# zwu88/TANTE

Hardware: AMD Instinct MI355X
Metric: rollout frames/sec (fwd), TANTE on 256x256 Active Matter (higher is better)
Workload: dtype bf16

## Files before the change

### include/tante_hip.h

```cpp
#ifndef TANTE_HIP_H
#define TANTE_HIP_H

#include <stddef.h>
#include <stdint.h>

#ifdef __cplusplus
extern "C" {
#endif

#define TANTE_F32 0
#define TANTE_BF16 1

#define TANTE_ACT_NONE 0
#define TANTE_ACT_GELU_ERF 1
#define TANTE_ACT_GELU_TANH 2
#define TANTE_ACT_RELU 3

#define TANTE_A_LINEAR 0
#define TANTE_A_PATCH_NHWC 1
#define TANTE_A_PATCH_NCHW 2

#define TANTE_E_LINEAR 0
#define TANTE_E_FILM 1
#define TANTE_E_DECONV_NHWC 2
// ... 101 lines not shown

int tante_taylor(const float* last, int64_t last_bstride, const float* const* derivs, int n_order, double dt,
                 int n_out, float* out, int64_t out_bstride, int64_t B, int64_t frame, void* stream);

int tante_rt_reduce(const float* t, int B, int L, float out_T, float ep, float* rt, void* stream);

int tante_block_fused_supported(int C, int n_head, int hidden, int L);
int64_t tante_block_stream_bytes(int C, int hidden);
int tante_pack_block(const float* ln1_w, const float* ln1_b, const float* in_w, const float* in_b, const float* out_w,
                     const float* out_b, const float* ln2_w, const float* ln2_b, const float* fc1_w, const float* fc1_b,
                     const float* fc2_w, const float* fc2_b, int C, int hidden, void* block_stream, void* stream);
int tante_block_fused(float* x, const void* block_stream, int C, int n_head, int hidden, const TanteSeq* seq, int causal,
                      float eps, void* stream);
int tante_block_fused_tprop(float* x, const void* block_stream, int C, int n_head, int hidden, const TanteSeq* seq, int causal, float eps,
                            const float* tprop, void* stream);

int tante_set_seed_mix(const uint64_t* device_word);

typedef struct TanteBlockTrain {
  float* out;
  void *xh1, *qkv, *o, *xh2, *hpre, *act;
  float *st1, *x1, *st2;
  float p_drop;
  uint64_t seed_attn, seed_out, seed_mlp;
} TanteBlockTrain;
int tante_pack_block_train(const float* in_w_folded, const float* in_b_folded, const float* out_w, const float* out_b,
                           const float* fc1_w_folded, const float* fc1_b_folded, const float* fc2_w, const float* fc2_b, int C, int hidden,
                           void* block_stream, void* stream);
int tante_block_fused_train(const float* x, const void* block_stream, int C, int n_head, int hidden, const TanteSeq* seq, int causal,
                            float eps, const TanteBlockTrain* tr, void* stream);
// ... 295 lines not shown
```

### tante_amd/_lib.py

```python
import ctypes as C
import os

HERE = os.path.dirname(os.path.abspath(__file__))
LIB_PATH = os.environ.get("TANTE_LIB") or os.path.join(HERE, "lib", "libtante_hip.so")

F32, BF16 = 0, 1
ACT_NONE, ACT_GELU_ERF, ACT_GELU_TANH, ACT_RELU = 0, 1, 2, 3
A_LINEAR, A_PATCH_NHWC, A_PATCH_NCHW = 0, 1, 2
E_LINEAR, E_FILM, E_DECONV_NHWC, E_DECONV_NCHW = 0, 1, 2, 3
W_LINEAR, W_CONV_NHWC, W_DECONV_NHWC, W_DECONV_NCHW = 0, 1, 2, 3
W_LINEAR_T, W_CONV_NHWC_T, W_DECONV_NHWC_T, W_DECONV_NCHW_T = 4, 5, 6, 7

c_i32, c_i64, c_f32, c_vp = C.c_int32, C.c_int64, C.c_float, C.c_void_p


class PackGeom(C.Structure):
    _fields_ = [("n_pad", c_i32), ("k_pad", c_i32), ("nt", c_i32), ("cb", c_i32), ("bytes", c_i64)]


class Gemm(C.Structure):
    _fields_ = [
        ("a", c_vp), ("a_dtype", c_i32), ("a_mode", c_i32), ("M", c_i32), ("K", c_i32),
        ("a_s1", c_i64), ("a_s0", c_i64), ("a_off", c_i64), ("a_n0", c_i32),
        ("Hin", c_i32), ("Win", c_i32), ("Cin", c_i32), ("P", c_i32), ("ln", c_i32), ("ln_eps", c_f32),
# ... 90 lines not shown
    "tante_axis_hw": ([c_vp, c_i64, c_i32, c_i32, c_i32] + [c_vp] * 8 + [c_i32, c_vp], c_i32),
    "tante_axis_hw_film": ([c_vp, c_vp, c_i64, c_i64, c_vp, c_vp, c_vp, c_i32, c_i64, c_i32, c_i32, c_i32] + [c_vp] * 8 + [c_i32, c_vp], c_i32),
    "tante_axis_hw_oop": ([c_vp, c_vp, c_i64, c_i32, c_i32, c_i32, c_vp, c_vp, c_vp, c_vp, c_vp, c_vp, c_vp, c_vp, c_i32, c_vp], c_i32),
    "tante_axis_hw_train": ([c_vp, c_vp, c_vp, c_i64, c_i32, c_i32, c_i32, c_vp, c_vp, c_vp, c_vp, c_vp, c_vp, c_vp, c_vp, c_i32, c_vp], c_i32),
    "tante_film_table": ([c_vp, c_i32, c_i32] + [c_vp] * 8 + [c_vp, c_vp, c_vp, c_vp], c_i32),
    "tante_film_apply": ([c_vp, c_i64, c_vp, c_i64, c_i32, c_i64, c_vp, c_vp, c_vp], c_i32),
    "tante_format_input": ([c_vp, c_i64, c_i32, c_i64, c_i32, c_vp, c_i64, c_vp], c_i32),
    "tante_taylor": ([c_vp, c_i64, C.POINTER(c_vp), c_i32, C.c_double, c_i32, c_vp, c_i64, c_i64, c_i64, c_vp], c_i32),
    "tante_rt_reduce": ([c_vp, c_i32, c_i32, c_f32, c_f32, c_vp, c_vp], c_i32),
    "tante_gather_last": ([c_vp, c_i64, c_i32, c_vp, c_vp], c_i32),
    "tante_block_fused_supported": ([c_i32, c_i32, c_i32, c_i32], c_i32),
    "tante_block_stream_bytes": ([c_i32, c_i32], c_i64),
    "tante_pack_block": ([c_vp] * 12 + [c_i32, c_i32, c_vp, c_vp], c_i32),
    "tante_block_fused": ([c_vp, c_vp, c_i32, c_i32, c_i32, C.POINTER(Seq), c_i32, c_f32, c_vp], c_i32),
    "tante_block_fused_tprop": ([c_vp, c_vp, c_i32, c_i32, c_i32, C.POINTER(Seq), c_i32, c_f32, c_vp, c_vp], c_i32),
    "tante_block_tail_bwd_stream_bytes": ([c_i32, c_i32], c_i64),
    "tante_pack_block_tail_bwd": ([c_vp, c_vp, c_vp, c_i32, c_i32, c_vp, c_vp], c_i32),
    "tante_block_tail_bwd": ([c_vp, c_vp, c_vp, c_vp, c_vp, c_i64, c_i32, c_i32, c_f32, C.c_uint64, C.c_uint64, c_vp, c_vp, c_vp, c_vp, c_vp, c_vp], c_i32),
    "tante_block_head_bwd": ([c_vp, c_vp, c_vp, c_vp, c_vp, c_i64, c_i32, c_vp, c_vp], c_i32),
    "tante_block_bwd_fused_supported": ([c_i32, c_i32, c_i32, c_i32, c_i32], c_i32),
    "tante_block_bwd_fused": ([c_vp] * 9 + [c_i32, c_i32, c_i32, C.POINTER(Seq), c_i32, c_f32, C.c_uint64, C.c_uint64, C.c_uint64] + [c_vp] * 6, c_i32),
    "tante_pack_block_train": ([c_vp] * 8 + [c_i32, c_i32, c_vp, c_vp], c_i32),
    "tante_block_fused_train": ([c_vp, c_vp, c_i32, c_i32, c_i32, C.POINTER(Seq), c_i32, c_f32, C.POINTER(BlockTrain), c_vp], c_i32),
    "tante_head_fused_supported": ([c_i32, c_i32], c_i32),
    "tante_head_stream_bytes": ([c_i32], c_i64),
    "tante_pack_head": ([c_vp] * 6 + [c_i32, c_i32, c_vp, c_vp], c_i32),
    "tante_head_fused": ([c_vp, c_i32, c_i64, c_i64, c_i64, c_i32, c_i32, c_i32, c_i32, c_i32, c_vp, c_vp, c_i64, c_i32, c_vp, c_vp, c_i64, c_vp], c_i32),
    "tante_enc23_supported": ([c_i32], c_i32),
    "tante_enc23_stream_bytes": ([c_i32], c_i64),
    "tante_pack_enc23": ([c_vp] * 4 + [c_i32, c_vp, c_vp], c_i32),
# ... 93 lines not shown
    "tante_pack_head_enc": ([c_vp] * 6 + [c_i32, c_i32, c_vp, c_vp], c_i32),
    "tante_head_enc_fused": ([c_i32, c_vp, c_vp, c_vp, c_i32, c_i64, c_i64, c_i64, c_i32, c_i32, c_i32, c_i32, c_i32, c_vp, c_i64, c_vp, c_i64,
                             c_vp, c_vp, c_vp, c_i64, c_vp], c_i32),
}

LIB_OPTIONS = ("TANTE_ATTN_BWD_HG", "TANTE_ATTN_BWD_NO_SPLIT", "TANTE_ATTN_BWD_VALU", "TANTE_ATTN_FWD_VALU", "TANTE_AXIS_BWD_SMALL_WGS",
               "TANTE_AXIS_BWD_WGS", "TANTE_AXIS_CT", "TANTE_AXIS_FILM", "TANTE_AXIS_GENERIC", "TANTE_AXIS_MFMA", "TANTE_AXIS_NT", "TANTE_AXIS_WGRAD_WGS",
               "TANTE_BLOCK_KERNEL", "TANTE_COLSUM_ROWS", "TANTE_CVIT_CHAIN_TOKENS", "TANTE_ENC23_SPLIT", "TANTE_FILM_BWD_ROWS",
               "TANTE_FS_GROUPS", "TANTE_FS_HALF", "TANTE_FS_SKEW", "TANTE_FS_WAVES", "TANTE_GEMM_NO_LITE", "TANTE_GEMM_SMALLM", "TANTE_GEMM_WGS", "TANTE_HEAD_WAVES",
               "TANTE_IM2COL_TILED", "TANTE_RESIZE_TILED", "TANTE_SPECTRAL_BF16OUT", "TANTE_SPECTRAL_DFT", "TANTE_SPECTRAL_X3", "TANTE_WGRAD_DEEP",
               "TANTE_WGRAD_JOBS", "TANTE_WGRAD_JOBS_WGS", "TANTE_WGRAD_NO_SLAB", "TANTE_WGRAD_NO_TR", "TANTE_WGRAD_REDUCE_NY",
               "TANTE_WGRAD_RG", "TANTE_WGRAD_SLAB_WGS", "TANTE_WGRAD_TR_WGS", "TANTE_WGRAD_WGS", "TANTE_XATTN_GPW", "TANTE_XATTN_VALU",)


_lib = None
ABI_VERSION = 12


def lib():
    global _lib
    if _lib is None:
        if not os.path.exists(LIB_PATH):
            raise RuntimeError(
                f"{LIB_PATH} is missing: build it with `python -m tante_amd.build` "
                "(or __graft_entry__.build()).  tante_amd has no CPU / eager fallback.")
        L = C.CDLL(LIB_PATH)
        for name, (argtypes, restype) in SIGNATURES.items():
            fn = getattr(L, name)
            fn.argtypes = argtypes
            fn.restype = restype
        got = int(L.tante_abi_version())
# ... 32 lines not shown
```

### tante_amd/attn_backbone.py

```python
from __future__ import annotations

import math
import os
from typing import Optional

import torch
import torch.nn as nn

from . import _lib as L
from . import kernels as K
from . import options as _O

FUSE_TPROP = _O.register("TANTE_FUSE_TPROP", True, __name__, "FUSE_TPROP")


def resolve_compute(module_default: Optional[str] = None) -> int:
    if module_default is not None:
        return K.COMPUTE[module_default]
    if torch.is_autocast_enabled("cuda"):
        dt = torch.get_autocast_dtype("cuda")
        if dt == torch.bfloat16:
            return L.BF16
        if dt == torch.float16:
            global _FP16_NOTED
# ... 81 lines not shown
        params = self.__dict__.get("_fused_params")
        if params is None:
            a, m = self.attn, self.mlp
            params = [self.ln1.weight, self.ln1.bias, a.in_proj_weight, a.in_proj_bias, a.out_proj.weight, a.out_proj.bias,
                      self.ln2.weight, self.ln2.bias, m[0].weight, m[0].bias, m[2].weight, m[2].bias]
            self.__dict__["_fused_params"] = params
        return self._cache.get(-1, params, lambda: K.pack_block(params, self.embed_dim, self.hidden))

    def _apply(self, fn, *a, **kw):
        self.__dict__.pop("_fused_params", None)
        return super()._apply(fn, *a, **kw)

    def takes_tprop(self, seq_L: int, compute: int) -> bool:
        return (FUSE_TPROP and compute == L.BF16 and self.fused and self.ln1.eps == self.ln2.eps and seq_L == 4 and self.embed_dim == 256
                and self.n_head == 8 and self.hidden == 256 and not (self.training and self.p_drop > 0.0))

    def forward_tokens(self, x: torch.Tensor, seq: L.Seq, causal: bool, compute: int, tprop: Optional[torch.Tensor] = None) -> torch.Tensor:
        if self.training and self.p_drop > 0.0:
            if tprop is not None:
                raise RuntimeError("TransformerBlock.forward_tokens: tprop is an inference-path fusion (takes_tprop is False under dropout)")
            from .train_forward import block_train
            with torch.no_grad():
                y = block_train(self, x.view(-1, self.embed_dim), seq, causal, compute)
            x.view(-1, self.embed_dim).copy_(y)
            return x
        C_ = self.embed_dim
        n_tok = x.numel() // C_
        if (compute == L.BF16 and self.fused and self.ln1.eps == self.ln2.eps
                and K.block_fused_supported(C_, self.n_head, self.hidden, seq.L)):
            return K.block_fused(x, self._packed_fused(), C_, self.n_head, self.hidden, seq, causal, self.ln1.eps, tprop)
# ... 116 lines not shown
        tp = self.temporal_propagator
        params = [tp[0].weight, tp[0].bias, tp[2].weight, tp[2].bias]
        return self._tp_cache.get(0, params, lambda: torch.cat([p.detach().float().reshape(-1) for p in params]).contiguous())

    def _packed_channel(self, compute: int):
        params = [p for cb in self.channel_blocks for p in cb.parameters()]

        def build():
            return [(K.pack_weight(cb[0].weight, cb[0].bias, compute), K.pack_weight(cb[2].weight, cb[2].bias, compute))
                    for cb in self.channel_blocks]
        return self._cache.get(compute, params, build)

    def takes_x_in(self, compute: int) -> bool:
        return K.axis_hw_train_supported(self.H, self.W, self.C, compute)

    def forward_tokens(self, x: torch.Tensor, B: int, compute: int, film_src: Optional[tuple] = None, x_in: Optional[torch.Tensor] = None,
                       film_frames: Optional[tuple] = None) -> torch.Tensor:
        T, H, W, C_ = self.T, self.H, self.W, self.C
        vp, hp, tp = self.vertical_propagator, self.horizontal_propagator, self.temporal_propagator
        if film_frames is not None:
            import ctypes as C
            fr, _keep, fa, fb, se = film_frames
            L.check(L.lib().tante_axis_mlp_film(x.data_ptr(), C.byref(fr), fa.data_ptr(), fb.data_ptr(), se.data_ptr(), B, T, H, W * C_, C_,
                                                vp[0].weight.data_ptr(), vp[0].bias.data_ptr(), vp[2].weight.data_ptr(), vp[2].bias.data_ptr(),
                                                K._stream()), "tante_axis_mlp_film")
            K.axis_mlp(x, B * T * H, W, C_, hp[0].weight, hp[0].bias, hp[2].weight, hp[2].bias, compute)
        elif x_in is not None:
            K.axis_hw_oop(x_in, x, B * T, H, W, C_, (vp[0].weight, vp[0].bias, vp[2].weight, vp[2].bias),
                          (hp[0].weight, hp[0].bias, hp[2].weight, hp[2].bias), compute)
        elif film_src is not None:
            z, ts, bs, film = film_src
            K.axis_hw_film(x, z, ts, bs, film, B * T, H, W, C_, (vp[0].weight, vp[0].bias, vp[2].weight, vp[2].bias),
                           (hp[0].weight, hp[0].bias, hp[2].weight, hp[2].bias), compute)
        elif K.axis_hw_supported(H, W, C_, compute):
            K.axis_hw(x, B * T, H, W, C_, (vp[0].weight, vp[0].bias, vp[2].weight, vp[2].bias),
                      (hp[0].weight, hp[0].bias, hp[2].weight, hp[2].bias), compute)
        else:
            K.axis_mlp(x, B * T, H, W * C_, vp[0].weight, vp[0].bias, vp[2].weight, vp[2].bias, compute)
            K.axis_mlp(x, B * T * H, W, C_, hp[0].weight, hp[0].bias, hp[2].weight, hp[2].bias, compute)
        tprop = None
        if (T == 4 and len(self.attn_axes) > 0 and self.attn_axes[0] == "T" and not torch.is_grad_enabled()
                and self.blocks[0].takes_tprop(T, compute)):
            tprop = self._packed_tprop()
        else:
            K.axis_mlp(x, B, T, H * W * C_, tp[0].weight, tp[0].bias, tp[2].weight, tp[2].bias, compute)
        ci = 0
        for i, axis in enumerate(self.attn_axes):
            blk = self.blocks[i]
            if axis == "C":
                E = self.expanded_channel
                lift1, lift2 = self._packed_channel(compute)[ci]
                ci += 1
                n = x.numel()
                adt = K.act_torch_dtype(compute)
                z1 = torch.empty(n, E // 4, dtype=adt, device=x.device)
                K.linear(x, lift1, z1, M=n, act=L.ACT_GELU_ERF, a_s0=1)
                z = torch.empty(n, E, dtype=torch.float32, device=x.device)
                K.linear(z1, lift2, z, M=n)
                blk.forward_tokens(z, K.dense_seq(n // C_, C_), False, compute)
                K.gather_last(z, n, E, x)
            else:
                blk.forward_tokens(x, K.make_seq(axis, B, T, H, W), axis == "T", compute, tprop if i == 0 else None)
        return x

# ... 12 lines not shown
```

### tante_amd/csrc/block_fused.hip

```cpp
#include "common.hip.h"

#include <stdlib.h>
#include "fused_common.hip.h"
#include "block_sliced.h"

namespace {

constexpr int BIAS_BYTES = 4096;

__device__ __forceinline__ long seq_token(const TanteSeq& q, int s, int l) {
  return (long)(s / q.n_s0) * q.S1 + (long)(s % q.n_s0) * q.S0 + (long)(l / q.n_l0) * q.P1 + (long)(l % q.n_l0) * q.P0;
}

template <int BYTES>
__device__ __forceinline__ void glds_copy(const char* __restrict__ g, char* l, int tid) {
  static_assert(BYTES % 4096 == 0, "tiles are whole LDS-DMA passes");
  const int wave = tid >> 6, lane = tid & 63;
#pragma unroll
  for (int i = 0; i < BYTES / 4096; ++i) {
    const int off = i * 4096 + wave * 1024;
    __builtin_amdgcn_global_load_lds((const __attribute__((address_space(1))) void*)(g + off + lane * 16),
                                     (__attribute__((address_space(3))) void*)(l + off), 16, 0, 0);
  }
}
// ... 676 lines not shown
  return 0;
}

extern "C" int tante_block_fused_tprop(float* x, const void* block_stream, int C, int n_head, int hidden, const TanteSeq* seq, int causal, float eps,
                                       const float* tprop, void* stream) {
  if (!x || !block_stream || !seq || !tprop) TANTE_FAIL(-1, "tante_block_fused_tprop: null pointer");
  if (seq->L != 4 || !tante_block_fused_supported(C, n_head, hidden, seq->L) || !use_fs(C, n_head, hidden, seq->L, causal))
    TANTE_FAIL(-2, "tante_block_fused_tprop: the feature-sliced kernel at L = 4 only (C=%d heads=%d hidden=%d L=%d)", C, n_head, hidden, seq->L);
  if (((uintptr_t)x % 16) || ((uintptr_t)block_stream % 16)) TANTE_FAIL(-1, "tante_block_fused_tprop: buffers must be 16-byte aligned");
  if (tante_fs_launch(x, (const char*)block_stream + block_ts_stream_bytes(C, hidden), *seq, causal, eps, (hipStream_t)stream, nullptr, tprop) != 0)
    TANTE_FAIL(-2, "tante_block_fused_tprop: too many sequences (%d)", seq->nseq);
  TANTE_CHECK_LAUNCH();
  return 0;
}

extern "C" int tante_block_fused(float* x, const void* block_stream, int C, int n_head, int hidden, const TanteSeq* seq, int causal,
                                 float eps, void* stream) {
  if (!x || !block_stream || !seq) TANTE_FAIL(-1, "tante_block_fused: null pointer");
  if (!tante_block_fused_supported(C, n_head, hidden, seq->L))
    TANTE_FAIL(-2, "tante_block_fused: unsupported shape C=%d heads=%d hidden=%d L=%d", C, n_head, hidden, seq->L);
  if (((uintptr_t)x % 16) || ((uintptr_t)block_stream % 16)) TANTE_FAIL(-1, "tante_block_fused: buffers must be 16-byte aligned");
  hipStream_t s = (hipStream_t)stream;
  const char* st = (const char*)block_stream;
  if (use_fs(C, n_head, hidden, seq->L, causal)) {
    if (tante_fs_launch(x, st + block_ts_stream_bytes(C, hidden), *seq, causal, eps, s) != 0)
      TANTE_FAIL(-2, "tante_block_fused: too many sequences (%d)", seq->nseq);
    TANTE_CHECK_LAUNCH();
    return 0;
  }
  const int key = (C / 32) * 100 + hidden / 32;
// ... 60 lines not shown
```

### tante_amd/csrc/block_sliced.h

```cpp
#pragma once
#include <hip/hip_runtime.h>
#include <stdint.h>
#include "../../include/tante_hip.h"

int tante_fs_supported(int C, int n_head, int hidden, int L, int causal);
int64_t tante_fs_stream_bytes(int C, int hidden);
void tante_fs_pack(const float* ln1_w, const float* ln1_b, const float* in_w, const float* in_b, const float* out_w, const float* out_b,
                   const float* ln2_w, const float* ln2_b, const float* fc1_w, const float* fc1_b, const float* fc2_w,
                   const float* fc2_b, char* dst, hipStream_t s);
void tante_fs_pack_folded(const float* in_w, const float* in_b, const float* out_w, const float* out_b, const float* fc1_w,
                          const float* fc1_b, const float* fc2_w, const float* fc2_b, char* dst, hipStream_t s);
constexpr int TANTE_FSP_MAX = 12;
void tante_fs_pack_folded_multi(const float* const (*params)[8], char* const* dst, int n, hipStream_t s);
int tante_fs_launch(float* x, const char* stream, const TanteSeq& sq, int causal, float eps, hipStream_t s, const TanteBlockTrain* tr = nullptr,
                    const float* tprop = nullptr);
```

### tante_amd/csrc/block_sliced.hip

```cpp
#include "common.hip.h"
#include "fused_common.hip.h"
#include "fs_common.hip.h"
#include "block_sliced.h"

#if (defined(FS_EXP_NO_SAVE) || defined(FS_EXP_LN_ID) || defined(FS_EXP_GELU_ID) || defined(FS_EXP_NO_RESID) || defined(FS_EXP_NO_STORE) || \
     defined(FS_EXP_TPROP_NO_STORE) || defined(FS_EXP_ROT) || defined(FS_EXP_NO_WLOAD) || defined(FS_EXP_MFMA32)) && !defined(TANTE_ABLATE)
#error "FS_EXP_* timing experiments produce wrong results on purpose: build them with -DTANTE_ABLATE (tools/build_variant.sh), never into the product library"
#endif

namespace {


struct FsArgs {
  float* x;
  const char* w;
  TanteSeq sq;
  int causal;
  float eps;
  int spw;
  unsigned magic;
  float* out;
  unsigned short *xh1, *qkv, *o, *xh2, *hpre, *act;
  float *st1, *x1, *st2;
  float p_drop;
// ... 65 lines not shown
#pragma unroll
    for (int j = 0; j < 4; ++j) acc = __builtin_amdgcn_mfma_f32_4x4x1f32(w.w2c[j], hid[e][j], acc, 0, 0, 0);
    yy[e] = acc;
  }
#pragma unroll
  for (int t = 0; t < 4; ++t) xs[t] = f32x4{yy[0][t], yy[1][t], yy[2][t], yy[3][t]};
}

constexpr int fs_group(int ntt, int nk) {
  int g = 1;
  for (int d = 1; d <= ntt; ++d)
    if (ntt % d == 0 && d * nk <= 8) g = d;
  return g;
}

template <int TPS, int NTT, int NW, bool TRAIN, int G = 1, bool TPROP = false>
__global__ __launch_bounds__(64 * NW * G, 2) void block_fs_kernel(FsArgs A) {
  static_assert(!TPROP || (TPS == 1 && !TRAIN), "the fused temporal propagator: T letter (L = 4), inference");
  static_assert(G == 1 || (G == 2 && NW == 4), "the paired form is two 4-wave groups");
  constexpr int RT = 16 / NW;
  constexpr int HPW = RT / 2;
#ifndef FS_PF8
#define FS_PF8 3
#endif
#ifndef FS_PF4
#define FS_PF4 2
#endif
#ifdef FS_NO_TIGHT
  constexpr bool TIGHT = false;
#else
  constexpr bool TIGHT = (NW == 4 && NTT == 4 && (TRAIN || TPS == 0)) || (NW == 8 && NTT == 8);
#endif
  constexpr int PF = (NW == 8 ? FS_PF8 : FS_PF4) - (TIGHT ? 1 : 0);
// ... 111 lines not shown
    }
  };
  auto slice_store = [&](float* __restrict__ dst, const f32x4 (&acc)[RT][NTT]) {
#pragma unroll
    for (int tt = 0; tt < NTT; ++tt) {
      char* sb = stg + (tt % NSUB) * TILEB;
#pragma unroll
      for (int rt = 0; rt < RT; ++rt) *(f32x4*)(sb + l15 * ROWB + (((4 * rt + kk) ^ (l15 & (CPR - 1))) << 4)) = acc[rt][tt];
#pragma unroll
      for (int j = 0; j < RT; ++j) {
        const int r = RPI * j + rrow, t = tok_of(16 * tt + r);
        const f32x4 v = *(const f32x4*)(sb + r * ROWB + ((rchunk ^ (r & (CPR - 1))) << 4));
#ifdef FS_NT_STORE
        if (t >= 0) __builtin_nontemporal_store(v, (f32x4*)(dst + (long)t * FS_C + 16 * RT * wave + 4 * rchunk));
#else
        if (t >= 0) {
          if constexpr (TRAIN) *(f32x4*)(dst + (long)t * FS_C + 16 * RT * wave + 4 * rchunk) = v;
          else st_wt16(dst + (long)t * FS_C + 16 * RT * wave + 4 * rchunk, v);
        }
#endif
      }
    }
  };

  constexpr bool ln1_done = TPROP;
  if constexpr (TPROP) {
    {
      constexpr int GPW = 4 * NTT / NW;
      f32x4 xv[GPW][4];
#pragma unroll
      for (int i = 0; i < GPW; ++i)
// ... 3 lines not shown
          xv[i][t] = *(const f32x4*)(x + (long)(tk < 0 ? 0 : tk) * FS_C + 4 * lane);
        }
      fs_wring_prime<0, RT, PF>(wq, wb);
      TpropW tw;
      tprop_weights(A.tprop, lane, tw);
#pragma unroll
      for (int i = 0; i < GPW; ++i) {
        tprop_apply(tw, xv[i]);
#pragma unroll
        for (int t = 0; t < 4; ++t) {
          const f32x4 y = xv[i][t];
          const int tk = tok_of(4 * (wave * GPW + i) + t);
          const bool live = tk >= 0;
#ifndef FS_TPROP_RECOMPUTE
#ifndef FS_EXP_TPROP_NO_STORE
          if (live) *(f32x4*)(x + (long)tk * FS_C + 4 * lane) = y;
#endif
#endif
          float sm = (y[0] + y[1]) + (y[2] + y[3]);
          float sq = fmaf(y[0], y[0], fmaf(y[1], y[1], fmaf(y[2], y[2], y[3] * y[3])));
          sm = rows_sum(row16_sum(sm));
          sq = rows_sum(row16_sum(sq));
          const float mean = sm * (1.0f / FS_C);
          const float var = fmaxf(sq * (1.0f / FS_C) - mean * mean, 0.0f);
          const float rstd = live ? rsqrtf(var + A.eps) : 0.0f;
          const float sh = live ? -mean * rstd : 0.0f;
          const int slot = 4 * (wave * GPW + i) + t;
          u32x2 o2;
          o2[0] = pack_bf16x2(fmaf(y[0], rstd, sh), fmaf(y[1], rstd, sh));
          o2[1] = pack_bf16x2(fmaf(y[2], rstd, sh), fmaf(y[3], rstd, sh));
          *(u32x2*)(bufA + slot * FS_ROW + (((lane >> 1) ^ (slot & 15)) << 4) + (lane & 1) * 8) = o2;
// ... 602 lines not shown
                               const float* __restrict__ be2, const float* __restrict__ w2, const float* __restrict__ b2,
                               char* __restrict__ dst) {
  fs_pack_body((int)blockIdx.x, w_in, b_in, g1, be1, w_out, b_out, w1, b1, g2, be2, w2, b2, dst);
}
constexpr int FSP_BLOCKS = FS_W_BYTES / FS_FRAG / 4 + 1;
struct FsPackBatch {
  const float* p[TANTE_FSP_MAX][8];
  char* dst[TANTE_FSP_MAX];
};
__global__ void fs_pack_multi_kernel(FsPackBatch B) {
  const int e = blockIdx.x / FSP_BLOCKS;
  const float* const* q = B.p[e];
  fs_pack_body((int)blockIdx.x - e * FSP_BLOCKS, q[0], q[1], nullptr, nullptr, q[2], q[3], q[4], q[5], nullptr, nullptr, q[6], q[7], B.dst[e]);
}

template <int TPS, int NTT, int NW, bool TRAIN, int G = 1, bool TPROP = false>
void fs_launch_tt(const FsArgs& A, int nwg, hipStream_t s) {
  constexpr int LDS = G * (2 * 16 * NTT * FS_ROW + 16 * NTT * NW * 8 + FS_BIAS_FLOATS * 4);
  static_assert(LDS <= 160 * 1024, "LDS per workgroup");
  static TantePerDevice attr;
  attr.once([&] { (void)hipFuncSetAttribute((const void*)block_fs_kernel<TPS, NTT, NW, TRAIN, G, TPROP>, hipFuncAttributeMaxDynamicSharedMemorySize, LDS); });
  hipLaunchKernelGGL((block_fs_kernel<TPS, NTT, NW, TRAIN, G, TPROP>), dim3((nwg + G - 1) / G), dim3(64 * NW * G), LDS, s, A);
}
template <int TPS, int NTT, int NW>
void fs_launch_t(const FsArgs& A, int nwg, hipStream_t s) {
  if constexpr (NW == 4) {
    if (A.out) return fs_launch_tt<TPS, NTT, NW, true>(A, nwg, s);
    if constexpr (TPS == 1) {
      if (A.tprop) return fs_launch_tt<TPS, NTT, NW, false, 1, true>(A, nwg, s);
    }
    const int groups = tante_opt("TANTE_FS_GROUPS", 0);
    if (groups == 2) return fs_launch_tt<TPS, NTT, NW, false, 2>(A, nwg, s);
  }
  fs_launch_tt<TPS, NTT, NW, false>(A, nwg, s);
}

int fs_waves(int L) {
// ... 25 lines not shown
                          const float* fc1_b, const float* fc2_w, const float* fc2_b, char* dst, hipStream_t s) {
  hipLaunchKernelGGL(fs_pack_kernel, dim3(FS_W_BYTES / FS_FRAG / 4 + 1), dim3(256), 0, s, in_w, in_b, (const float*)nullptr,
                     (const float*)nullptr, out_w, out_b, fc1_w, fc1_b, (const float*)nullptr, (const float*)nullptr, fc2_w, fc2_b, dst);
}

void tante_fs_pack_folded_multi(const float* const (*params)[8], char* const* dst, int n, hipStream_t s) {
  FsPackBatch B;
  for (int e = 0; e < n; ++e) {
    for (int k = 0; k < 8; ++k) B.p[e][k] = params[e][k];
    B.dst[e] = dst[e];
  }
  hipLaunchKernelGGL(fs_pack_multi_kernel, dim3((unsigned)(n * FSP_BLOCKS)), dim3(256), 0, s, B);
}

int tante_fs_launch(float* x, const char* stream, const TanteSeq& sq, int causal, float eps, hipStream_t s, const TanteBlockTrain* tr,
                    const float* tprop) {
  if (sq.nseq >= (1 << 23)) return -2;
  if (tprop && (tr || sq.L != 4)) return -5;
  FsArgs A;
  A.x = x; A.w = stream; A.sq = sq; A.causal = causal; A.eps = eps;
  A.out = nullptr;
  A.seed_mix = nullptr;
  A.tprop = tprop;
  if (tr) {
    if (sq.L > 64) return -4;
    A.out = tr->out; A.xh1 = (unsigned short*)tr->xh1; A.st1 = tr->st1; A.qkv = (unsigned short*)tr->qkv; A.o = (unsigned short*)tr->o;
    A.x1 = tr->x1; A.xh2 = (unsigned short*)tr->xh2; A.st2 = tr->st2; A.hpre = (unsigned short*)tr->hpre; A.act = (unsigned short*)tr->act;
    A.p_drop = tr->p_drop; A.seed_attn = tr->seed_attn; A.seed_out = tr->seed_out; A.seed_mlp = tr->seed_mlp;
    A.seed_mix = tante_seed_mix_ptr();
  }
  A.stamps = nullptr;
#ifdef TANTE_ABLATE
  A.stamps = g_fs_stamps;
#endif
  const int L = sq.L, nw = (tr || tprop) ? 4 : fs_waves(L);
  A.magic = (65536u + (unsigned)L - 1u) / (unsigned)L;
  int tps = 0;
  if (16 % L == 0) tps = 1;
  else if (!causal && (L == 32 || L == 48 || L == 64)) tps = L / 16;
  const int full = nw == 8 ? 8 : 4, tq = nw == 8 ? 6 : 3;
  const long resident = 256L * (8 / nw);
  auto rounds = [&](int ntt) {
    const int spw = 16 * ntt / L;
    const long nwg = (sq.nseq + spw - 1) / spw;
    return ((nwg + resident - 1) / resident) * ntt;
  };
  int ntt = full;
  if (tps == 3) ntt = tq;
  else if (tps >= 1 && (16 * tq) % L == 0 && (16 * tq) / L >= 1 && (tps == 1 || tq % tps == 0) && rounds(tq) < rounds(full)) ntt = tq;
  if (!tr && nw == 4 && (tps == 1 || tps == 2) && 32 % L == 0 && tante_opt("TANTE_FS_HALF", 1)) {
    const int spw_full = 16 * ntt / L;
    if (((long)sq.nseq + spw_full - 1) / spw_full * 4 <= resident) ntt = 2;
  }
  A.spw = tps ? 16 * ntt / L : (16 * full) / L;
  const int nwg = (sq.nseq + A.spw - 1) / A.spw;
  A.skew = (!tr && nw == 4 && nwg > 256 && nwg <= 512) ? tante_opt("TANTE_FS_SKEW", 0) : 0;
  const int key = nw * 100 + tps * 10 + ntt;
  switch (key) {
    case 412:
      if (A.tprop) fs_launch_tt<1, 2, 4, false, 1, true>(A, nwg, s);
      else fs_launch_tt<1, 2, 4, false>(A, nwg, s);
      break;
    case 422: fs_launch_tt<2, 2, 4, false>(A, nwg, s); break;
    case 818: fs_launch_t<1, 8, 8>(A, nwg, s); break;
    case 816: fs_launch_t<1, 6, 8>(A, nwg, s); break;
    case 828: fs_launch_t<2, 8, 8>(A, nwg, s); break;
    case 826: fs_launch_t<2, 6, 8>(A, nwg, s); break;
    case 836: fs_launch_t<3, 6, 8>(A, nwg, s); break;
    case 848: fs_launch_t<4, 8, 8>(A, nwg, s); break;
    case 808: fs_launch_t<0, 8, 8>(A, nwg, s); break;
    case 414: fs_launch_t<1, 4, 4>(A, nwg, s); break;
// ... 10 lines not shown
```

### tante_amd/csrc/pointwise.hip

```cpp
#include "common.hip.h"
#include <stdlib.h>
#include <string.h>
#include <mutex>
#include <algorithm>

int tante_axis_mlp_mfma_supported(int64_t outer, int n, int64_t inner, const void* x, const void* w1, const void* w2);
int tante_axis_mlp_mfma(float* x, int64_t outer, int n, int64_t inner, const float* w1, const float* b1, const float* w2, const float* b2, hipStream_t s);

namespace {

template <int N>
__global__ __launch_bounds__(256) void axis_mlp_kernel(float* __restrict__ x, long outer, int n, long inner,
                                                       const float* __restrict__ w1, const float* __restrict__ b1,
                                                       const float* __restrict__ w2, const float* __restrict__ b2) {
  __shared__ __attribute__((aligned(16))) float w1s[N * N];
  __shared__ __attribute__((aligned(16))) float w2ts[N * N];
  __shared__ __attribute__((aligned(16))) float b1s[N];
  __shared__ __attribute__((aligned(16))) float b2s[N];
  for (int idx = threadIdx.x; idx < N * N; idx += 256) {
    const int j = idx / N, a = idx % N;
    const bool in = (j < n) && (a < n);
    w1s[idx] = in ? w1[j * n + a] : 0.0f;
    w2ts[idx] = in ? w2[a * n + j] : 0.0f;
  }
// ... 1120 lines not shown
    if (!strcmp(g_opts[i].name, name)) return g_opts[i].value;
  return dflt;
}
extern "C" int tante_set_option(const char* name, int value) {
  if (!name || !*name || strlen(name) >= sizeof(g_opts[0].name)) TANTE_FAIL(-1, "tante_set_option: bad option name");
  if (strncmp(name, "TANTE_", 6)) TANTE_FAIL(-1, "tante_set_option: option names start with TANTE_ (got '%s')", name);
  std::lock_guard<std::mutex> lk(g_opt_mutex);
  for (int i = 0; i < g_nopts; ++i)
    if (!strcmp(g_opts[i].name, name)) { g_opts[i].value = value; return 0; }
  if (g_nopts == TANTE_OPT_MAX) TANTE_FAIL(-1, "tante_set_option: table full");
  strcpy(g_opts[g_nopts].name, name);
  g_opts[g_nopts++].value = value;
  return 0;
}
extern "C" int tante_get_option(const char* name, int dflt) { return name ? tante_opt(name, dflt) : dflt; }
extern "C" int tante_abi_version(void) { return 12; }
```

### tante_amd/kernels.py

```python
from __future__ import annotations

import ctypes as C
from typing import Optional, Sequence, Tuple

import torch

from . import _lib as L

_DT = {torch.float32: L.F32, torch.bfloat16: L.BF16}
COMPUTE = {"fp32": L.F32, "float32": L.F32, "bf16": L.BF16, "bfloat16": L.BF16}


def _stream() -> int:
    return torch._C._cuda_getCurrentRawStream(torch._C._cuda_getDevice())


def _dev(*ts):
    for t in ts:
        if t is None:
            continue
        if not t.is_cuda:
            raise RuntimeError("tante_amd kernels need CUDA/HIP tensors (no CPU fallback)")
        if not t.is_contiguous():
            raise RuntimeError("tante_amd kernels need contiguous tensors")
# ... 143 lines not shown
    elif letter == "W":
        s.nseq, s.L, s.n_s0, s.S1, s.S0, s.n_l0, s.P1, s.P0 = B * T * H, W, 1, W, 0, W, 0, 1
    elif letter == "L":
        s.nseq, s.L, s.n_s0, s.S1, s.S0, s.n_l0, s.P1, s.P0 = B * T, HW, 1, HW, 0, HW, 0, 1
    elif letter == "Y":
        s.nseq, s.L, s.n_s0, s.S1, s.S0, s.n_l0, s.P1, s.P0 = B * W, T * H, W, THW, 1, H, HW, W
    elif letter == "X":
        s.nseq, s.L, s.n_s0, s.S1, s.S0, s.n_l0, s.P1, s.P0 = B * H, T * W, H, THW, W, W, HW, 1
    elif letter == "A":
        s.nseq, s.L, s.n_s0, s.S1, s.S0, s.n_l0, s.P1, s.P0 = B, THW, 1, THW, 0, THW, 0, 1
    else:
        raise ValueError(f"invalid axis letter {letter!r}")
    return s


def dense_seq(nseq: int, Lq: int) -> L.Seq:
    s = L.Seq()
    s.nseq, s.L, s.n_s0, s.S1, s.S0, s.n_l0, s.P1, s.P0 = nseq, Lq, 1, Lq, 0, Lq, 0, 1
    return s


def attention(qkv: torch.Tensor, o: torch.Tensor, C_: int, n_head: int, seq: L.Seq, causal: bool):
    _dev(qkv, o)
    if qkv.dtype != o.dtype:
        raise RuntimeError("qkv and o must share a dtype")
    L.check(L.lib().tante_attention(_p(qkv), _p(o), _DT[qkv.dtype], C_, n_head, C.byref(seq), int(causal), _stream()),
            "tante_attention")
    return o


# ... 121 lines not shown
    st = torch.empty(L.lib().tante_block_stream_bytes(C_, hidden), dtype=torch.uint8, device=ps[0].device)
    L.check(L.lib().tante_pack_block(*[_p(p) for p in ps], C_, hidden, _p(st), _stream()), "tante_pack_block")
    return st


def block_fused(x: torch.Tensor, block_stream: torch.Tensor, C_: int, n_head: int, hidden: int, seq: L.Seq, causal: bool,
                eps: float, tprop: Optional[torch.Tensor] = None):
    _dev(x, block_stream)
    if tprop is not None:
        _dev(tprop)
        L.check(L.lib().tante_block_fused_tprop(_p(x), _p(block_stream), C_, n_head, hidden, C.byref(seq), int(causal), eps, _p(tprop), _stream()),
                "tante_block_fused_tprop")
        return x
    L.check(L.lib().tante_block_fused(_p(x), _p(block_stream), C_, n_head, hidden, C.byref(seq), int(causal), eps, _stream()),
            "tante_block_fused")
    return x


def block_fused_train_supported(C_: int, n_head: int, hidden: int, Lq: int) -> bool:
    return C_ == 256 and n_head == 8 and hidden == 256 and 1 <= Lq <= 64


def pack_block_train(params: Sequence[torch.Tensor], C_: int, hidden: int) -> torch.Tensor:
    ps = [p.detach() for p in params]
    _dev(*ps)
    st = torch.empty(L.lib().tante_block_stream_bytes(C_, hidden), dtype=torch.uint8, device=ps[0].device)
    L.check(L.lib().tante_pack_block_train(*[_p(p) for p in ps], C_, hidden, _p(st), _stream()), "tante_pack_block_train")
    return st


# ... 346 lines not shown
```

### tante_amd/tante.py

```python
from __future__ import annotations

import ctypes as C
import math
from dataclasses import dataclass
from typing import Dict, List, Optional, Tuple

import torch
import torch.nn as nn

from . import _lib as L
from . import options as _O
from . import kernels as K
from . import stages as S
from .attn_backbone import Attn_Backbone, _PackCache, _gpu_only, _no_autograd, _wants_grad, resolve_compute

Patch_map = {64: (4, 4, 4), 32: (4, 4, 2), 16: (4, 2, 2), 8: (2, 2, 2), 4: (2, 2, 1), 2: (2, 1, 1)}


@dataclass
class TanteMetadata:
    dataset_name: str = "synthetic"
    n_spatial_dims: int = 2
    spatial_resolution: Tuple[int, ...] = (128, 384)
    field_names: Optional[Dict[int, List[str]]] = None
# ... 1 lines not shown
    n_files: int = 1
    n_trajectories_per_file: Optional[List[int]] = None
    n_steps_per_trajectory: Optional[List[int]] = None
    n_fields: int = 4

    @property
    def sample_shapes(self):
        return {"input_fields": [*self.spatial_resolution, self.n_fields],
                "output_fields": [*self.spatial_resolution, self.n_fields],
                "space_grid": [*self.spatial_resolution, self.n_spatial_dims]}


HEAD_MULTI = _O.register("TANTE_HEAD_MULTI", True, __name__, "HEAD_MULTI")
HEAD_STREAMS = _O.register("TANTE_HEAD_STREAMS", True, __name__, "HEAD_STREAMS")
HEAD_ENC = _O.register("TANTE_HEAD_ENC", True, __name__, "HEAD_ENC")


def _check_patch_cfg(patch_scale, overlap_ratio):
    if not 0.0 <= overlap_ratio < 1.0:
        raise AssertionError("overlap_ratio must be in [0, 1).")
    return Patch_map[patch_scale]


def _film_pos(v: torch.Tensor, film: tuple) -> torch.Tensor:
    fa, fb, se, T, HW = film
    y = torch.empty_like(v)
    L.check(L.lib().tante_film_pos_fwd(v.data_ptr(), fa.data_ptr(), fb.data_ptr(), se.data_ptr(), v.shape[0], v.shape[1], T, HW, y.data_ptr(),
                                       K._stream()), "tante_film_pos_fwd")
    return y

# ... 469 lines not shown
            if not self.deg:
                raise ValueError("out= is only meaningful with a fixed output length (deg=True)")
            if tuple(out.shape) != (B, self.output_length, D, H, W) or out.dtype != torch.float32 or not out.is_cuda \
                    or out.stride()[1:] != (frame, H * W, W, 1) or out.stride(0) % 4 or out.data_ptr() % 16:
                raise ValueError("out must be a (B, output_length, D, H, W) fp32 CUDA view with contiguous frames")
        derivs, r_t, srcs = [], [], []
        tail_fused = self.tail_fused_supported()
        if enc_next is not None:
            if not tail_fused or not self.encoder.fuses_23(compute):
                raise RuntimeError("enc_next: this model / compute mode has no fused head + re-encoding path (tail_fused_supported())")
            if tuple(enc_next.shape) != (B, HW, C_) or enc_next.dtype != torch.float32 or not enc_next.is_cuda or not enc_next.is_contiguous():
                raise ValueError("enc_next must be a contiguous (B, Hp*Wp, C) fp32 CUDA tensor")
        multi_head = (self.deg and fused_head and self.output_length == 1 and 2 <= self.taylor_order <= 4 and HEAD_MULTI) or tail_fused
        saved_rows = []
        streams = tail_fused or (multi_head and HEAD_STREAMS and all(b.takes_x_in(compute) for b in self.blocks[1:self.taylor_order]))
        for i in range(self.taylor_order):
            if streams and i > 0:
                x_prev, x = x, torch.empty_like(x)
                self.blocks[i].forward_tokens(x, B, compute, x_in=x_prev)
            else:
                self.blocks[i].forward_tokens(x, B, compute, film_src=(enc_cache + (film,)) if (enc_cache is not None and i == 0) else None,
                                              film_frames=film_frames if i == 0 else None)
            if self.deg:
                if multi_head:
                    if i + 1 < self.taylor_order:
                        saved_rows.append(x if streams else
                                          x.view(B, T, HW * C_)[:, T - 1].clone(memory_format=torch.contiguous_format).view(B * HW, C_))
                        continue
                    if out is None:
                        out = torch.empty(B, 1, D, H, W, dtype=torch.float32, device=x.device)
                    coefs = [self.frame_interval ** (k + 1) / math.factorial(k + 1) for k in range(self.taylor_order)]
                    if tail_fused:
                        K.head_enc_fused(saved_rows + [x], HW, T * HW * C_, C_, (T - 1) * HW * C_, B, Hp, Wp, C_, D,
                                         [self.decoders[k].packed_head() for k in range(self.taylor_order)], coefs, out, out.stride(0),
                                         inp, (T - 1) * frame, bstride,
                                         enc_stream=self.encoder.packed_head_enc() if enc_next is not None else None, z=enc_next)
                        continue
# ... 42 lines not shown
```

Baseline: 18080.

## Compute only the last time slot in the final Taylor-order block

In the final backbone block of an inference rollout with output length 1, only the last time slot feeds the head. This adds a last-slot variant of the feature-sliced T-axis kernel that writes back only the t=3 rows. The spatial-axis blocks that follow then run on that single slot's subgrid, which skips attention and MLP work on the other three slots. The cost is extra planning logic and new kernel template instances, and the path is gated on specific shapes and axis orders.

```diff
diff --git a/include/tante_hip.h b/include/tante_hip.h
--- a/include/tante_hip.h
+++ b/include/tante_hip.h
@@ -139,6 +139,9 @@
                       float eps, void* stream);
 int tante_block_fused_tprop(float* x, const void* block_stream, int C, int n_head, int hidden, const TanteSeq* seq, int causal, float eps,
                             const float* tprop, void* stream);
+int tante_block_fused_last_supported(int C, int n_head, int hidden, int L);
+int tante_block_fused_last(float* x, const void* block_stream, int C, int n_head, int hidden, const TanteSeq* seq, int causal, float eps,
+                           const float* tprop, void* stream);
 
 int tante_set_seed_mix(const uint64_t* device_word);
 
diff --git a/tante_amd/_lib.py b/tante_amd/_lib.py
--- a/tante_amd/_lib.py
+++ b/tante_amd/_lib.py
@@ -128,6 +128,8 @@
     "tante_pack_block": ([c_vp] * 12 + [c_i32, c_i32, c_vp, c_vp], c_i32),
     "tante_block_fused": ([c_vp, c_vp, c_i32, c_i32, c_i32, C.POINTER(Seq), c_i32, c_f32, c_vp], c_i32),
     "tante_block_fused_tprop": ([c_vp, c_vp, c_i32, c_i32, c_i32, C.POINTER(Seq), c_i32, c_f32, c_vp, c_vp], c_i32),
+    "tante_block_fused_last_supported": ([c_i32, c_i32, c_i32, c_i32], c_i32),
+    "tante_block_fused_last": ([c_vp, c_vp, c_i32, c_i32, c_i32, C.POINTER(Seq), c_i32, c_f32, c_vp, c_vp], c_i32),
     "tante_block_tail_bwd_stream_bytes": ([c_i32, c_i32], c_i64),
     "tante_pack_block_tail_bwd": ([c_vp, c_vp, c_vp, c_i32, c_i32, c_vp, c_vp], c_i32),
     "tante_block_tail_bwd": ([c_vp, c_vp, c_vp, c_vp, c_vp, c_i64, c_i32, c_i32, c_f32, C.c_uint64, C.c_uint64, c_vp, c_vp, c_vp, c_vp, c_vp, c_vp], c_i32),
@@ -251,7 +253,7 @@
 
 
 _lib = None
-ABI_VERSION = 12
+ABI_VERSION = 13
 
 
 def lib():
diff --git a/tante_amd/attn_backbone.py b/tante_amd/attn_backbone.py
--- a/tante_amd/attn_backbone.py
+++ b/tante_amd/attn_backbone.py
@@ -119,6 +119,16 @@
     def takes_tprop(self, seq_L: int, compute: int) -> bool:
         return (FUSE_TPROP and compute == L.BF16 and self.fused and self.ln1.eps == self.ln2.eps and seq_L == 4 and self.embed_dim == 256
                 and self.n_head == 8 and self.hidden == 256 and not (self.training and self.p_drop > 0.0))
+
+    def fused_inference(self, seq_L: int, compute: int) -> bool:
+        return (compute == L.BF16 and self.fused and self.ln1.eps == self.ln2.eps and not (self.training and self.p_drop > 0.0)
+                and K.block_fused_supported(self.embed_dim, self.n_head, self.hidden, seq_L))
+
+    def forward_last_slot(self, x: torch.Tensor, seq: L.Seq, causal: bool, tprop: Optional[torch.Tensor] = None) -> torch.Tensor:
+        return K.block_fused_last(x, self._packed_fused(), self.embed_dim, self.n_head, self.hidden, seq, causal, self.ln1.eps, tprop)
+
+    def forward_subgrid(self, x: torch.Tensor, row0: int, seq: L.Seq, causal: bool) -> torch.Tensor:
+        return K.block_fused_subgrid(x, row0, self._packed_fused(), self.embed_dim, self.n_head, self.hidden, seq, causal, self.ln1.eps)
 
     def forward_tokens(self, x: torch.Tensor, seq: L.Seq, causal: bool, compute: int, tprop: Optional[torch.Tensor] = None) -> torch.Tensor:
         if self.training and self.p_drop > 0.0:
@@ -265,8 +275,21 @@
     def takes_x_in(self, compute: int) -> bool:
         return K.axis_hw_train_supported(self.H, self.W, self.C, compute)
 
+    def _last_slot_plan(self, B: int, compute: int) -> Optional[int]:
+        axes = self.attn_axes
+        j = max(axes.rfind(a) for a in "TYXA")
+        if j < 0 or axes[j] != "T" or self.T != 4 or torch.is_grad_enabled():
+            return None
+        blk = self.blocks[j]
+        if not (blk.fused_inference(self.T, compute) and K.block_fused_last_supported(blk.embed_dim, blk.n_head, blk.hidden, self.T)):
+            return None
+        for i in range(j + 1, len(axes)):
+            if axes[i] not in "HWL" or not self.blocks[i].fused_inference(K.last_slot_seq(axes[i], B, self.T, self.H, self.W).L, compute):
+                return None
+        return j
+
     def forward_tokens(self, x: torch.Tensor, B: int, compute: int, film_src: Optional[tuple] = None, x_in: Optional[torch.Tensor] = None,
-                       film_frames: Optional[tuple] = None) -> torch.Tensor:
+                       film_frames: Optional[tuple] = None, last_slot_only: bool = False) -> torch.Tensor:
         T, H, W, C_ = self.T, self.H, self.W, self.C
         vp, hp, tp = self.vertical_propagator, self.horizontal_propagator, self.temporal_propagator
         if film_frames is not None:
@@ -295,10 +318,15 @@
             tprop = self._packed_tprop()
         else:
             K.axis_mlp(x, B, T, H * W * C_, tp[0].weight, tp[0].bias, tp[2].weight, tp[2].bias, compute)
+        jl = self._last_slot_plan(B, compute) if last_slot_only else None
         ci = 0
         for i, axis in enumerate(self.attn_axes):
             blk = self.blocks[i]
-            if axis == "C":
+            if jl is not None and i == jl:
+                blk.forward_last_slot(x, K.make_seq(axis, B, T, H, W), True, tprop if i == 0 else None)
+            elif jl is not None and i > jl:
+                blk.forward_subgrid(x, (T - 1) * H * W, K.last_slot_seq(axis, B, T, H, W), False)
+            elif axis == "C":
                 E = self.expanded_channel
                 lift1, lift2 = self._packed_channel(compute)[ci]
                 ci += 1
diff --git a/tante_amd/csrc/block_fused.hip b/tante_amd/csrc/block_fused.hip
--- a/tante_amd/csrc/block_fused.hip
+++ b/tante_amd/csrc/block_fused.hip
@@ -714,6 +714,24 @@
   return 0;
 }
 
+extern "C" int tante_block_fused_last_supported(int C, int n_head, int hidden, int L) {
+  return C == 256 && n_head == 8 && hidden == 256 && L == 4 && use_fs(C, n_head, hidden, L, 0);
+}
+
+extern "C" int tante_block_fused_last(float* x, const void* block_stream, int C, int n_head, int hidden, const TanteSeq* seq, int causal,
+                                      float eps, const float* tprop, void* stream) {
+  if (!x || !block_stream || !seq) TANTE_FAIL(-1, "tante_block_fused_last: null pointer");
+  if (!tante_block_fused_last_supported(C, n_head, hidden, seq->L))
+    TANTE_FAIL(-2, "tante_block_fused_last: the feature-sliced kernel at C = 256 / 8 heads / hidden 256 / L = 4 only (C=%d heads=%d hidden=%d L=%d)",
+               C, n_head, hidden, seq->L);
+  if (((uintptr_t)x % 16) || ((uintptr_t)block_stream % 16)) TANTE_FAIL(-1, "tante_block_fused_last: buffers must be 16-byte aligned");
+  if (tante_fs_launch(x, (const char*)block_stream + block_ts_stream_bytes(C, hidden), *seq, causal, eps, (hipStream_t)stream, nullptr, tprop,
+                      true) != 0)
+    TANTE_FAIL(-2, "tante_block_fused_last: too many sequences (%d)", seq->nseq);
+  TANTE_CHECK_LAUNCH();
+  return 0;
+}
+
 extern "C" int tante_block_fused(float* x, const void* block_stream, int C, int n_head, int hidden, const TanteSeq* seq, int causal,
                                  float eps, void* stream) {
   if (!x || !block_stream || !seq) TANTE_FAIL(-1, "tante_block_fused: null pointer");
diff --git a/tante_amd/csrc/block_sliced.h b/tante_amd/csrc/block_sliced.h
--- a/tante_amd/csrc/block_sliced.h
+++ b/tante_amd/csrc/block_sliced.h
@@ -13,4 +13,4 @@
 constexpr int TANTE_FSP_MAX = 12;
 void tante_fs_pack_folded_multi(const float* const (*params)[8], char* const* dst, int n, hipStream_t s);
 int tante_fs_launch(float* x, const char* stream, const TanteSeq& sq, int causal, float eps, hipStream_t s, const TanteBlockTrain* tr = nullptr,
-                    const float* tprop = nullptr);
+                    const float* tprop = nullptr, bool lastq = false);
diff --git a/tante_amd/csrc/block_sliced.hip b/tante_amd/csrc/block_sliced.hip
--- a/tante_amd/csrc/block_sliced.hip
+++ b/tante_amd/csrc/block_sliced.hip
@@ -103,9 +103,10 @@
   return g;
 }
 
-template <int TPS, int NTT, int NW, bool TRAIN, int G = 1, bool TPROP = false>
+template <int TPS, int NTT, int NW, bool TRAIN, int G = 1, bool TPROP = false, bool LASTQ = false>
 __global__ __launch_bounds__(64 * NW * G, 2) void block_fs_kernel(FsArgs A) {
   static_assert(!TPROP || (TPS == 1 && !TRAIN), "the fused temporal propagator: T letter (L = 4), inference");
+  static_assert(!LASTQ || (TPS == 1 && NW == 4 && G == 1 && !TRAIN), "the last-slot form: T letter (L = 4), 4 waves, inference");
   static_assert(G == 1 || (G == 2 && NW == 4), "the paired form is two 4-wave groups");
   constexpr int RT = 16 / NW;
   constexpr int HPW = RT / 2;
@@ -247,7 +248,7 @@
 #ifdef FS_NT_STORE
         if (t >= 0) __builtin_nontemporal_store(v, (f32x4*)(dst + (long)t * FS_C + 16 * RT * wave + 4 * rchunk));
 #else
-        if (t >= 0) {
+        if (t >= 0 && (!LASTQ || (r & 3) == 3)) {
           if constexpr (TRAIN) *(f32x4*)(dst + (long)t * FS_C + 16 * RT * wave + 4 * rchunk) = v;
           else st_wt16(dst + (long)t * FS_C + 16 * RT * wave + 4 * rchunk, v);
         }
@@ -281,7 +282,7 @@
           const bool live = tk >= 0;
 #ifndef FS_TPROP_RECOMPUTE
 #ifndef FS_EXP_TPROP_NO_STORE
-          if (live) *(f32x4*)(x + (long)tk * FS_C + 4 * lane) = y;
+          if (live && (!LASTQ || t == 3)) *(f32x4*)(x + (long)tk * FS_C + 4 * lane) = y;
 #endif
 #endif
           float sm = (y[0] + y[1]) + (y[2] + y[3]);
@@ -914,13 +915,18 @@
   fs_pack_body((int)blockIdx.x - e * FSP_BLOCKS, q[0], q[1], nullptr, nullptr, q[2], q[3], q[4], q[5], nullptr, nullptr, q[6], q[7], B.dst[e]);
 }
 
-template <int TPS, int NTT, int NW, bool TRAIN, int G = 1, bool TPROP = false>
+template <int TPS, int NTT, int NW, bool TRAIN, int G = 1, bool TPROP = false, bool LASTQ = false>
 void fs_launch_tt(const FsArgs& A, int nwg, hipStream_t s) {
   constexpr int LDS = G * (2 * 16 * NTT * FS_ROW + 16 * NTT * NW * 8 + FS_BIAS_FLOATS * 4);
   static_assert(LDS <= 160 * 1024, "LDS per workgroup");
   static TantePerDevice attr;
-  attr.once([&] { (void)hipFuncSetAttribute((const void*)block_fs_kernel<TPS, NTT, NW, TRAIN, G, TPROP>, hipFuncAttributeMaxDynamicSharedMemorySize, LDS); });
-  hipLaunchKernelGGL((block_fs_kernel<TPS, NTT, NW, TRAIN, G, TPROP>), dim3((nwg + G - 1) / G), dim3(64 * NW * G), LDS, s, A);
+  attr.once([&] { (void)hipFuncSetAttribute((const void*)block_fs_kernel<TPS, NTT, NW, TRAIN, G, TPROP, LASTQ>, hipFuncAttributeMaxDynamicSharedMemorySize, LDS); });
+  hipLaunchKernelGGL((block_fs_kernel<TPS, NTT, NW, TRAIN, G, TPROP, LASTQ>), dim3((nwg + G - 1) / G), dim3(64 * NW * G), LDS, s, A);
+}
+template <int NTT>
+void fs_launch_last(const FsArgs& A, int nwg, hipStream_t s) {
+  if (A.tprop) fs_launch_tt<1, NTT, 4, false, 1, true, true>(A, nwg, s);
+  else fs_launch_tt<1, NTT, 4, false, 1, false, true>(A, nwg, s);
 }
 template <int TPS, int NTT, int NW>
 void fs_launch_t(const FsArgs& A, int nwg, hipStream_t s) {
@@ -976,9 +982,10 @@
 }
 
 int tante_fs_launch(float* x, const char* stream, const TanteSeq& sq, int causal, float eps, hipStream_t s, const TanteBlockTrain* tr,
-                    const float* tprop) {
+                    const float* tprop, bool lastq) {
   if (sq.nseq >= (1 << 23)) return -2;
   if (tprop && (tr || sq.L != 4)) return -5;
+  if (lastq && (tr || sq.L != 4)) return -5;
   FsArgs A;
   A.x = x; A.w = stream; A.sq = sq; A.causal = causal; A.eps = eps;
   A.out = nullptr;
@@ -995,7 +1002,7 @@
 #ifdef TANTE_ABLATE
   A.stamps = g_fs_stamps;
 #endif
-  const int L = sq.L, nw = (tr || tprop) ? 4 : fs_waves(L);
+  const int L = sq.L, nw = (tr || tprop || lastq) ? 4 : fs_waves(L);
   A.magic = (65536u + (unsigned)L - 1u) / (unsigned)L;
   int tps = 0;
   if (16 % L == 0) tps = 1;
@@ -1014,9 +1021,15 @@
     const int spw_full = 16 * ntt / L;
     if (((long)sq.nseq + spw_full - 1) / spw_full * 4 <= resident) ntt = 2;
   }
+  if (lastq && ntt == tq) ntt = full;
   A.spw = tps ? 16 * ntt / L : (16 * full) / L;
   const int nwg = (sq.nseq + A.spw - 1) / A.spw;
   A.skew = (!tr && nw == 4 && nwg > 256 && nwg <= 512) ? tante_opt("TANTE_FS_SKEW", 0) : 0;
+  if (lastq) {
+    if (ntt == 2) fs_launch_last<2>(A, nwg, s);
+    else fs_launch_last<4>(A, nwg, s);
+    return 0;
+  }
   const int key = nw * 100 + tps * 10 + ntt;
   switch (key) {
     case 412:
diff --git a/tante_amd/csrc/pointwise.hip b/tante_amd/csrc/pointwise.hip
--- a/tante_amd/csrc/pointwise.hip
+++ b/tante_amd/csrc/pointwise.hip
@@ -1158,4 +1158,4 @@
   return 0;
 }
 extern "C" int tante_get_option(const char* name, int dflt) { return name ? tante_opt(name, dflt) : dflt; }
-extern "C" int tante_abi_version(void) { return 12; }
+extern "C" int tante_abi_version(void) { return 13; }
diff --git a/tante_amd/kernels.py b/tante_amd/kernels.py
--- a/tante_amd/kernels.py
+++ b/tante_amd/kernels.py
@@ -181,6 +181,20 @@
     return s
 
 
+def last_slot_seq(letter: str, B: int, T: int, H: int, W: int) -> L.Seq:
+    s = L.Seq()
+    HW, THW = H * W, T * H * W
+    if letter == "H":
+        s.nseq, s.L, s.n_s0, s.S1, s.S0, s.n_l0, s.P1, s.P0 = B * W, H, W, THW, 1, H, 0, W
+    elif letter == "W":
+        s.nseq, s.L, s.n_s0, s.S1, s.S0, s.n_l0, s.P1, s.P0 = B * H, W, H, THW, W, W, 0, 1
+    elif letter == "L":
+        s.nseq, s.L, s.n_s0, s.S1, s.S0, s.n_l0, s.P1, s.P0 = B, HW, 1, THW, 0, HW, 0, 1
+    else:
+        raise ValueError(f"letter {letter!r} mixes time slots")
+    return s
+
+
 def dense_seq(nseq: int, Lq: int) -> L.Seq:
     s = L.Seq()
     s.nseq, s.L, s.n_s0, s.S1, s.S0, s.n_l0, s.P1, s.P0 = nseq, Lq, 1, Lq, 0, Lq, 0, 1
@@ -332,6 +346,28 @@
         return x
     L.check(L.lib().tante_block_fused(_p(x), _p(block_stream), C_, n_head, hidden, C.byref(seq), int(causal), eps, _stream()),
             "tante_block_fused")
+    return x
+
+
+def block_fused_last_supported(C_: int, n_head: int, hidden: int, Lq: int) -> bool:
+    return bool(L.lib().tante_block_fused_last_supported(C_, n_head, hidden, Lq))
+
+
+def block_fused_last(x: torch.Tensor, block_stream: torch.Tensor, C_: int, n_head: int, hidden: int, seq: L.Seq, causal: bool,
+                     eps: float, tprop: Optional[torch.Tensor] = None):
+    _dev(x, block_stream, tprop)
+    L.check(L.lib().tante_block_fused_last(_p(x), _p(block_stream), C_, n_head, hidden, C.byref(seq), int(causal), eps, _p(tprop), _stream()),
+            "tante_block_fused_last")
+    return x
+
+
+def block_fused_subgrid(x: torch.Tensor, row0: int, block_stream: torch.Tensor, C_: int, n_head: int, hidden: int, seq: L.Seq,
+                        causal: bool, eps: float):
+    _dev(x, block_stream)
+    if x.dtype != torch.float32 or row0 < 0 or row0 >= x.numel() // C_:
+        raise RuntimeError("block_fused_subgrid: fp32 stream and a row inside it")
+    L.check(L.lib().tante_block_fused(x.data_ptr() + row0 * C_ * 4, _p(block_stream), C_, n_head, hidden, C.byref(seq), int(causal), eps,
+                                      _stream()), "tante_block_fused")
     return x
 
 
diff --git a/tante_amd/tante.py b/tante_amd/tante.py
--- a/tante_amd/tante.py
+++ b/tante_amd/tante.py
@@ -39,6 +39,7 @@
 HEAD_MULTI = _O.register("TANTE_HEAD_MULTI", True, __name__, "HEAD_MULTI")
 HEAD_STREAMS = _O.register("TANTE_HEAD_STREAMS", True, __name__, "HEAD_STREAMS")
 HEAD_ENC = _O.register("TANTE_HEAD_ENC", True, __name__, "HEAD_ENC")
+LAST_SLOT = _O.register("TANTE_LAST_SLOT", True, __name__, "LAST_SLOT")
 
 
 def _check_patch_cfg(patch_scale, overlap_ratio):
@@ -538,13 +539,15 @@
         multi_head = (self.deg and fused_head and self.output_length == 1 and 2 <= self.taylor_order <= 4 and HEAD_MULTI) or tail_fused
         saved_rows = []
         streams = tail_fused or (multi_head and HEAD_STREAMS and all(b.takes_x_in(compute) for b in self.blocks[1:self.taylor_order]))
+        slot_only = LAST_SLOT and self.deg and multi_head and self.output_length == 1 and not torch.is_grad_enabled()
         for i in range(self.taylor_order):
+            ls = slot_only and i + 1 == self.taylor_order
             if streams and i > 0:
                 x_prev, x = x, torch.empty_like(x)
-                self.blocks[i].forward_tokens(x, B, compute, x_in=x_prev)
+                self.blocks[i].forward_tokens(x, B, compute, x_in=x_prev, last_slot_only=ls)
             else:
                 self.blocks[i].forward_tokens(x, B, compute, film_src=(enc_cache + (film,)) if (enc_cache is not None and i == 0) else None,
-                                              film_frames=film_frames if i == 0 else None)
+                                              film_frames=film_frames if i == 0 else None, last_slot_only=ls)
             if self.deg:
                 if multi_head:
                     if i + 1 < self.taylor_order:
```

New measurement: 19800, median of 6. 1.1x the previous value.
